# zhouxuguang/GNXRayTracer

Hardware: AMD Instinct MI355X
Metric: Mrays/sec + wall-clock to 1024spp, dragon Cornell 1920×1080 (higher is better)
Workload: dtype f32; 1 GPU; cfg3: Cornell + synthetic 100000-tri mesh (stand-in for absent dragon.3d), Glass+Metal, PathIntegrator maxDepth 8 rr 1 spatial, Halton(1024), 1920x1080; passes_in_flight=4, sub_passes=56, spp_rendered=1024, gather=n/a, world_size=1, backend=none, devices_visible=1

## Files before the change

gnxraytracer_amd/csrc/api_query.hip.h:

```cpp
#pragma once

extern "C" {


static const long long kQueryLaunchMax = 1ll << 30;

static DScene query_device_scene(gnxr_scene *r) {
    const CompiledScene &cs = r->cs;
    DScene sc = {};
    sc.nodes = reinterpret_cast<const float4 *>(r->nodes.p);
    sc.nodes4 = reinterpret_cast<const float4 *>(r->nodes4.p);
    sc.root4 = cs.root4;
    sc.tris = r->tris.p;
    sc.leaf_box = reinterpret_cast<const float4 *>(r->leaf_boxes.p);
    sc.leaf1_from_verts = (cs.leaf1_from_verts && !Knobs::leaf_box_table()) ? 1 : 0;
    sc.spheres = r->spheres.p;
    sc.n_spheres = cs.n_spheres;
    sc.materials = r->materials.p + 1;
    return sc;
}

static int query_trace4(gnxr_scene *r, const DScene &sc, const gnxr_ray *d_rays, int64_t n, gnxr_hit *hits, unsigned char *occluded, bool any, hipStream_t st) {
    const bool spheres = r->cs.n_spheres > 0;
    const TraceLaunch tl = trace_launch(r, true, spheres, std::min<long long>(n, kQueryLaunchMax));
    const size_t spill_ints = tl.spill_needed ? (size_t)(tl.entries - tl.lds_entries) * (size_t)tl.blocks * kBlock : 0;
    StreamScratch scratch;
    HIP_TRY(scratch.alloc(256 + spill_ints * sizeof(int), st));
    unsigned int *cursor = reinterpret_cast<unsigned int *>(scratch.p);
    int *spill = reinterpret_cast<int *>(scratch.p + 256);
    for (long long base = 0; base < n; base += kQueryLaunchMax) {
        const long long cnt = std::min<long long>(n - base, kQueryLaunchMax);
        const TraceLaunch t = trace_launch(r, true, spheres, cnt);
        QueryArrays qa;
        qa.rays = reinterpret_cast<const float4 *>(d_rays + base);
        qa.hits = any ? nullptr : hits + base;
        qa.occluded = any ? occluded + base : nullptr;
        TraceWork w = {};
        w.n_closest = (int)cnt;
        HIP_TRY(hipMemsetAsync(cursor, 0, sizeof(unsigned int), st));
#define GX_QUERY4(S, P, Q) hipLaunchKernelGGL((k_trace4<false, S, P, Q>), dim3(t.blocks), dim3(kBlock), t.lds, st, sc, qa, w, cursor, (Counters *)nullptr, t.lds_entries, spill, kTraceChunk, t.n_top)
#define GX_QUERY4_SP(Q) do { if (spheres) { if (t.spill_needed) GX_QUERY4(true, true, Q); else GX_QUERY4(true, false, Q); } \
                             else { if (t.spill_needed) GX_QUERY4(false, true, Q); else GX_QUERY4(false, false, Q); } } while (0)
        if (any) GX_QUERY4_SP(kT4QueryAny);
        else GX_QUERY4_SP(kT4QueryClosest);
#undef GX_QUERY4_SP
#undef GX_QUERY4
        HIP_TRY(hipGetLastError());
    }
    return GNXR_OK;
}

static int closest_hit_codes(gnxr_scene *r, const DScene &sc, const gnxr_ray *d_rays, long long n, gnxr_hit *codes, hipStream_t st) {
    if (r->wide_ok) return query_trace4(r, sc, d_rays, n, codes, nullptr, false, st);
    if (r->stack_size > 32) hipLaunchKernelGGL((k_trace_closest_code<64>), dim3(grid_for(n, 2)), dim3(kBlock), 0, st, sc, d_rays, n, codes);
    else hipLaunchKernelGGL((k_trace_closest_code<32>), dim3(grid_for(n, 5)), dim3(kBlock), 0, st, sc, d_rays, n, codes);
    HIP_TRY(hipGetLastError());
    return GNXR_OK;
}

static int trace_device(gnxr_scene *s, const gnxr_ray *d_rays, int64_t n, void *out, void *hip_stream, bool any) {
    if (!s || n < 0 || (n > 0 && (!d_rays || !out))) { set_error("bad argument"); return GNXR_ERR_INVALID; }
    if (n == 0) return GNXR_OK;
    if (((uintptr_t)d_rays & 15u) != 0) { set_error("d_rays is not 16-byte aligned (two dwordx4 loads per ray)"); return GNXR_ERR_INVALID; }
    if (!any && ((uintptr_t)out & 3u) != 0) { set_error("d_hits is not 4-byte aligned"); return GNXR_ERR_INVALID; }
    const QueryArg args[] = {{d_rays, (size_t)n * sizeof(gnxr_ray), "d_rays"}, {out, (size_t)n * (!any ? sizeof(gnxr_hit) : 1), !any ? "d_hits" : "d_occluded"}};
    DeviceCall call;
    int rc = call.bind(s, args);
    if (rc) return rc;
    gnxr_scene *r = call.r;
    hipStream_t st = (hipStream_t)hip_stream;
    const DScene sc = query_device_scene(r);
    if (!r->wide_ok) return binary_trace_api(r, sc, d_rays, n, out, any, st);
    if ((rc = query_trace4(r, sc, d_rays, n, any ? nullptr : (gnxr_hit *)out, any ? (unsigned char *)out : nullptr, any, st)) != GNXR_OK) return rc;
    if (!any) {
        hipLaunchKernelGGL(k_query_finish, dim3(grid_for(n)), dim3(kBlock), 0, st, sc, reinterpret_cast<const float4 *>(d_rays), (long long)n, (gnxr_hit *)out);
        HIP_TRY(hipGetLastError());
    }
    return GNXR_OK;
}
int gnxr_trace_closest_device(gnxr_scene *s, const gnxr_ray *d_rays, int64_t n, gnxr_hit *d_hits, void *hip_stream) {
    return trace_device(s, d_rays, n, d_hits, hip_stream, false);
}
int gnxr_trace_any_device(gnxr_scene *s, const gnxr_ray *d_rays, int64_t n, uint8_t *d_occluded, void *hip_stream) {
    return trace_device(s, d_rays, n, d_occluded, hip_stream, true);
}

int gnxr_li_device(gnxr_scene *s, const gnxr_render_params *p, const gnxr_ray *d_rays, const gnxr_li_sample *d_samples, int64_t n, float *d_L, void *hip_stream,
                   gnxr_stats *stats) {
    if (int rc = ensure_device()) return rc;
    if (!s || !p || n < 0 || (n > 0 && (!d_rays || !d_samples || !d_L))) { set_error("bad argument"); return GNXR_ERR_INVALID; }
    if (p->spp_begin != 0 || p->spp_end != 0) { set_error("Li for caller rays: spp_begin and spp_end must be 0 (the records name each ray's sample)"); return GNXR_ERR_INVALID; }
    if (int rc = check_unsharded(*p, "Li for caller rays", "the records name each ray's sample")) return rc;
    if (n == 0) { if (stats) memset(stats, 0, sizeof(*stats)); return GNXR_OK; }
    if ((((uintptr_t)d_rays | (uintptr_t)d_samples | (uintptr_t)d_L) & 15u) != 0) { set_error("d_rays, d_samples and d_L must be 16-byte aligned"); return GNXR_ERR_INVALID; }
    const QueryArg args[] = {{d_rays, (size_t)n * sizeof(gnxr_ray), "d_rays"}, {d_samples, (size_t)n * sizeof(gnxr_li_sample), "d_samples"}, {d_L, (size_t)n * 4 * sizeof(float), "d_L"}};
    DeviceCall call;
    if (int rc = call.bind(s, args)) return rc;
    gnxr_render_params pp = *p;
    pp.shard_count = 1; pp.shard_rows = 1;
    const RaySource src{d_rays, d_samples, d_L, (long long)n};
    return render_one(call.r, &pp, nullptr, hip_stream, stats, false, &src);
}

int gnxr_render_views_device(gnxr_scene *s, const gnxr_render_params *p, const gnxr_camera *cameras, const int32_t *camera_media, int32_t n_views, void *d_rgba_out,
                             void *hip_stream, gnxr_stats *stats) {
    if (!s || !p || n_views < 0 || (n_views > 0 && !cameras)) { set_error("bad argument"); return GNXR_ERR_INVALID; }
    if (int rc = check_unsharded(*p, "views", "a caller that shards splits the list of views")) return rc;
    if (!image_and_samples_ok(*p) || p->max_depth < 0 || p->max_depth > 250) return invalid_render_params();
    if (n_views == 0) { if (stats) memset(stats, 0, sizeof(*stats)); return GNXR_OK; }
    if (!d_rgba_out || ((uintptr_t)d_rgba_out & 15u) != 0) { set_error("d_rgba_out is null or not 16-byte aligned"); return GNXR_ERR_INVALID; }
    long long total = 0;
    if (int rc = check_view_pixels(p->width, p->height, n_views, "views", &total)) return rc;
    if (int rc = ensure_device()) return rc;
    if (int rc = check_view_media(s, camera_media, n_views, "views")) return rc;
    const QueryArg args[] = {{d_rgba_out, (size_t)total * sizeof(float4), "d_rgba_out"}};
    DeviceCall call;
    if (int rc = call.bind(s, args)) return rc;
    gnxr_render_params pp = *p;
    pp.shard_count = 1; pp.shard_rows = 1;
    const ViewSource vs{cameras, camera_media, (int)n_views};
    return render_one(call.r, &pp, d_rgba_out, hip_stream, stats, false, nullptr, &vs);
}


static const long long kBsdfQueryChunk = 1ll << 22;
// ... 94 lines not shown
```

gnxraytracer_amd/csrc/api_render.hip.h:

```cpp
#pragma once

struct TraceLaunch {
    int entries;
    int lds_entries;
    bool spill_needed;
    size_t lds;
    int n_top;
    int blocks;
};
static TraceLaunch trace_launch(const gnxr_scene *s, bool wide, bool spheres, long long total) {
    TraceLaunch t;
    t.entries = wide ? s->cs.stack4_need + 1 : s->cs.bvh_max_depth + 2;
    const int per_cu = g_trace_blocks_per_cu;
    const size_t fixed_b = wide ? (size_t)(kRayRecDwords + (spheres ? 1 : 0)) * kRqStride * sizeof(int) + (size_t)kTopCache * 128 + kOrderTableBytes : 0;
    t.lds_entries = std::min(std::min(t.entries, Knobs::trace_lds_levels()), std::max(2, (int)(((160 * 1024) / per_cu - 1024 - fixed_b) / (kBlock * sizeof(int)))));
    t.spill_needed = t.entries > t.lds_entries;
    t.lds = (size_t)t.lds_entries * kBlock * sizeof(int) + fixed_b;
    t.n_top = (int)std::min<size_t>(kTopCache, s->cs.root4 >= 0 ? s->cs.nodes4.size() : 0);
    t.blocks = (int)std::min<long long>((long long)g_num_cus * per_cu, (total + kBlock - 1) / kBlock);
    return t;
}

static int count_local_rows(const gnxr_render_params *p) {
    int rows = 0;
    for (int y = 0; y < p->height; ++y)
        if ((y / p->shard_rows) % p->shard_count == p->shard_index) ++rows;
    return rows;
}

struct RaySource {
    const gnxr_ray *rays;
    const gnxr_li_sample *samples;
    float *L;
    long long n;
};

struct ViewSource {
    const gnxr_camera *cameras;
    const int32_t *media;
    int n_views;
};

struct FilmSource {
    FilmFilter f;
    FilmTable tab;
    float4 *accum;
    bool keep;
};

static FilmImage film_image(int W, int H, int n_views) {
    FilmImage im;
    im.W = W; im.H = H;
    im.npix = (long long)n_views * W * H;
    im.tiles_x = (W + kFilmTile - 1) / kFilmTile;
    im.tiles_y = (H + kFilmTile - 1) / kFilmTile;
    im.n_tiles = (long long)n_views * im.tiles_y * im.tiles_x;
    return im;
}
static int film_grid(const FilmImage &im) { return grid_for(im.n_tiles * kBlock, 32); }

struct PixelListSource {
    gnxr_adaptive_params ap;
    int32_t *count_out;
    PixelRound round;
    int rounds;
    long long samples, at_budget;
};

constexpr int kAdaptiveGrowth = 8;
static int adaptive_round_samples(const gnxr_adaptive_params &ap, int spp, int n0) {
    return n0 == 0 ? ap.min_spp : std::min(std::max(ap.step_spp, n0 / kAdaptiveGrowth), spp - n0);
}

struct RenderPlan {
    gnxr_render_params p;
    bool direct, volpath, whitted;
    int wmode;
    int n_records, max_light_samples;
    bool textured_scene;
    int class_mask;
    bool area_only, area_env_only;
    bool escape_queue;
    int queue_kernel[4];
    unsigned kind_queue;
    bool caller_rays;
    int n_views;
    bool pixel_list;
    int local_rows, npix;
    long long unit, unit_begin, unit_end;
    int spill_entries;
    int k, in_flight;
    size_t half, cap, nrec;

    bool path_int() const { return !whitted && !volpath; }
    int nsamples() const { return p.spp_end - p.spp_begin; }
    int size_passes(size_t slots_held, bool have_mem, size_t free_b);
};

enum ShadeQueueKernel { SHADE_Q_NONE = 0, SHADE_Q_DIFFUSE, SHADE_Q_GLOSSY, SHADE_Q_CONDUCTOR, SHADE_Q_ROUGH_DIELECTRIC, SHADE_Q_ALL, SHADE_Q_TEX, SHADE_Q_ESCAPE };
// ... 211 lines not shown
    va.bind_records(rec_primary);
    va.mis_Y = mis_Y.p;
    va.vs = vol_vs.p; va.n1 = vol_n1.p; va.f = vol_f.p;
    va.Li = vol_Li.p; va.Tr = vol_Tr.p; va.Ld = vol_Ld.p; va.mres = vol_mres.p; va.state = vol_state.p;
    va.orig = vol_orig.p; va.Lout = vol_Lout.p;
    return va;
}
WhittedArrays RenderState::whitted_arrays(const RenderPlan &pl, int n_lights) {
    WhittedArrays wa;
    wa.ws = vol_vs.p; wa.fr_o = wh_o.p; wa.fr_d = wh_d.p; wa.fr_L = wh_L.p; wa.fr_w = wh_w.p; wa.fr_pdf = wh_pdf.p;
    wa.fr_rxo = wh_rxo.p; wa.fr_rxd = wh_rxd.p; wa.fr_ryo = wh_ryo.p; wa.fr_ryd = wh_ryd.p;
    wa.cap = (int)pl.cap; wa.n_lights = n_lights; wa.n_records = pl.n_records;
    wa.start_dim = pl.wmode == WM_DIRECT_ALL ? 5 + 2 * (pl.p.max_depth * n_lights * 2) : 5;
    return wa;
}
VolPackSet RenderState::pack_set(bool alt) {
    VolPackSet ps;
    if (!alt) {
        float4 *a[kVolPackF4] = {L.p, reinterpret_cast<float4 *>(vol_vs.p), vol_n1.p, vol_f.p, vol_Li.p, vol_Tr.p, vol_Ld.p, mis_Y.p, vol_mres.p};
        for (int i = 0; i < kVolPackF4; ++i) ps.f4[i] = a[i];
        record_ptrs(rec, ps.rec);
        ps.state = vol_state.p; ps.orig = vol_orig.p;
    } else {
        for (int i = 0; i < kVolPackF4; ++i) ps.f4[i] = vol_alt[i].p;
        record_ptrs(vol_alt_rec, ps.rec);
        ps.state = vol_alt_state.p; ps.orig = vol_alt_orig.p;
    }
    return ps;
}

struct RenderRun {
    gnxr_scene *s;
    RenderState &st;
    hipStream_t stream;
    const RenderPlan &pl;
    const RaySource *src;
    const ViewSource *views;
    const PixelListSource *pix;
    const FilmSource *film = nullptr;
    float4 *film_accum = nullptr;
    DScene sc;
    DRender r;
    PathArrays pa;
    VolArrays va;
    WhittedArrays wa;
    DMediaTables mt;
    Counters *dctr;
    KernelTimer timer;
    const bool timing = (g_profiling & 1) != 0, count_wide = (g_profiling & 4) != 0, counting = (g_profiling & 2) != 0 && !count_wide;
    bool spheres;
    const int mis_mode = Knobs::no_mis_defer() ? 0 : Knobs::mis_defer_step(), mis_drain_at = Knobs::mis_defer_drain_at();
    bool list_media = false;
    int n_lights, n_scene_media;
    unsigned long long rays_closest = 0, rays_any = 0, rays_mis = 0, media_segments = 0;
    unsigned long long new_paths = 0;
    unsigned int launches = 0, passes = 0, loop_iterations = 0;

    RenderRun(gnxr_scene *scene, hipStream_t stream_, const RenderPlan &plan, const RaySource *src_, const ViewSource *views_, const PixelListSource *pix_, const DScene &sc_,
              const DRender &r_)
        : s(scene), st(scene->st), stream(stream_), pl(plan), src(src_), views(views_), pix(pix_), sc(sc_), r(r_), pa(st.path_arrays()), va(st.vol_arrays()),
          wa(st.whitted_arrays(plan, (int)scene->cs.desc_lights.size())), mt(scene->media_tables()), dctr(scene->counters.p), spheres(scene->cs.n_spheres > 0),
          n_lights((int)scene->cs.desc_lights.size()), n_scene_media((int)scene->cs.media.size()) {}

    void launch_trace(TraceWork w, int n_sh, int n_mis, bool count_rays = true);
    void compact(int mode, const int *qin, int nin, const unsigned char *keys, int nout, int nscatter, unsigned int *totals, int *o0, int *o1, int *o2, int *o3 = nullptr, int split = 0,
                 const unsigned *n_dev = nullptr, unsigned kind_queue = 0x01010101u);
    int shade_stage(const int *q_in, int n, int *q_out, const unsigned *n_dev);
    void raygen(const PathArrays &at, long long u0, int kk, unsigned char *medium_keys);
    void resolve(const PathArrays &at, long long u0, int kk);
    void bind_set(const VolPackSet &ps);
};

void RenderRun::launch_trace(TraceWork w, int n_sh, int n_mis, bool count_rays) {
    long long total = (long long)w.n_closest + w.n_nee;
    if (total <= 0) return;
    w.order = nullptr;
    (void)hipMemsetAsync(&dctr->cursor, 0, sizeof(unsigned int), stream);
    const bool wide = s->wide_ok && !counting;
    const TraceLaunch tl = trace_launch(s, wide, spheres, total);
    if (timing) timer.begin(0, stream);
    const int chunk = Knobs::trace_chunk();
#define GX_TRACE(C, W, S) hipLaunchKernelGGL((k_trace<C, W, S>), dim3(tl.blocks), dim3(kBlock), tl.lds, stream, sc, pa, w, &dctr->cursor, dctr, tl.lds_entries, st.trace_spill.p, chunk)
#define GX_TRACE4(C, S, P) hipLaunchKernelGGL((k_trace4<C, S, P>), dim3(tl.blocks), dim3(kBlock), tl.lds, stream, sc, pa, w, &dctr->cursor, dctr, tl.lds_entries, st.trace_spill.p, chunk, tl.n_top)
#define GX_TRACE4_CS(C, S) do { if (tl.spill_needed) GX_TRACE4(C, S, true); else GX_TRACE4(C, S, false); } while (0)
    if (wide) {
        if (spheres) { if (count_wide) GX_TRACE4_CS(true, true); else GX_TRACE4_CS(false, true); }
        else { if (count_wide) GX_TRACE4_CS(true, false); else GX_TRACE4_CS(false, false); }
    } else {
        const bool cnt = counting || count_wide;
        if (spheres) { if (cnt) GX_TRACE(true, false, true); else GX_TRACE(false, false, true); }
        else { if (cnt) GX_TRACE(true, false, false); else GX_TRACE(false, false, false); }
    }
#undef GX_TRACE4_CS
#undef GX_TRACE4
#undef GX_TRACE
    if (timing) timer.end(stream);
    if (count_rays) {
        rays_closest += (unsigned long long)w.n_closest + (unsigned long long)n_mis;
        rays_any += (unsigned long long)n_sh;
        rays_mis += (unsigned long long)n_mis;
    }
    ++launches;
}

void RenderRun::compact(int mode, const int *qin, int nin, const unsigned char *keys, int nout, int nscatter, unsigned int *totals, int *o0, int *o1, int *o2, int *o3, int split,
                        const unsigned *n_dev, unsigned kind_queue) {
    const int tiles = (nin + kCompactTile - 1) / kCompactTile;
    const int g = std::max(1, std::min(tiles, g_num_cus * kCompactBlocksPerCu));
    if (st.compact_seq >= (1u << 30) - 1u) {
        (void)hipMemsetAsync(st.tile_desc.p, 0, st.tile_desc.n * sizeof(unsigned long long), stream);
        st.compact_seq = 0;
    }
    const unsigned seq = ++st.compact_seq;
    const CompactScratch cs{st.tile_desc.p, tiles, st.compact_ticket.p + (seq & 1u), st.compact_ticket.p + ((seq + 1u) & 1u), seq};
    const bool hitclass = mode == COMPACT_HITCLASS;
    const int *hit = hitclass ? (const int *)st.hit.p : nullptr;
    const unsigned char *cls = hitclass ? (const unsigned char *)s->tri_class.p : nullptr;
#define GX_COMPACT(M, N, NS) hipLaunchKernelGGL((k_compact<M, N, NS>), dim3(g), dim3(kCompactBlock), 0, stream, qin, nin, keys, cs, totals, o0, o1, o2, o3, hit, cls, kind_queue, split, n_dev, dctr)
    if (mode == COMPACT_FLAGS) {
        if (nout == 5) { if (nscatter == 3) GX_COMPACT(COMPACT_FLAGS, 5, 3); else GX_COMPACT(COMPACT_FLAGS, 5, 2); }
        else { if (nscatter == 3) GX_COMPACT(COMPACT_FLAGS, 4, 3); else GX_COMPACT(COMPACT_FLAGS, 4, 2); }
    } else if (hitclass) { if (nout == 4) GX_COMPACT(COMPACT_HITCLASS, 4, 4); else GX_COMPACT(COMPACT_HITCLASS, 3, 3); }
    else if (nout == 4) GX_COMPACT(COMPACT_CLASS, 4, 4);
    else GX_COMPACT(COMPACT_CLASS, 3, 3);
#undef GX_COMPACT
    launches += 1;
}
static int compact_stalled(const Counters &c) {
    if (!c.compact_stall) return GNXR_OK;
    set_error("queue compaction: a tile waited for its predecessors beyond the poll limit (k_compact); the render was abandoned");
    return GNXR_ERR_RUNTIME;
}

constexpr size_t kShadeLdsBudget = 52 * 1024;

int RenderRun::shade_stage(const int *q_in, int n, int *q_out, const unsigned *n_dev) {
    if (timing) timer.begin(2, stream);
    const int *qk = pl.queue_kernel;
    const int n_classes = qk[3] != SHADE_Q_NONE ? 4 : 3;
    compact(COMPACT_HITCLASS, q_in, n, st.pclass.p, n_classes, n_classes, &dctr->q_class[0], st.queue_c0.p, st.queue_c1.p, st.queue_c2.p, st.queue_c3.p, 0, n_dev, pl.kind_queue);
    int *qc[4] = {st.queue_c0.p, st.queue_c1.p, st.queue_c2.p, st.queue_c3.p};
    dim3 g(grid_for(n, Knobs::shade_blocks_per_cu())), b(kBlock);
    const int sdims = std::min<int>(Knobs::shade_lds_dims(), (int)s->cs.prime_sums.size() - 1);
    const int snperm = sdims > 0 ? s->cs.prime_sums[sdims] : 0;
    const bool shade_lds_tabs = Knobs::shade_lds_tables();
    const int lmats = (shade_lds_tabs && s->cs.materials.size() <= 12) ? (int)s->cs.materials.size() : 0;
    const int llights = (shade_lds_tabs && n_lights > 0 && n_lights <= 16) ? n_lights : 0;
    const size_t slds = (sdims > 0 ? ((((size_t)snperm * 2 + 15) & ~(size_t)15) + (size_t)sdims * 32) : 0) + (size_t)lmats * sizeof(DMaterial) + (size_t)llights * sizeof(DLight);
    const int shade_streams = Knobs::shade_streams();
    int n_class_kernels = 0;
    for (int q = 0; q < 4; ++q) n_class_kernels += qk[q] != SHADE_Q_NONE ? 1 : 0;
    const bool fork = (shade_streams < 0 ? n_class_kernels >= 3 : (shade_streams != 0 && n_class_kernels >= 2)) && s->aux_stream[0] && s->aux_stream[1];
    hipStream_t cst[4] = {stream, stream, stream, stream};
    if (fork) {
        HIP_TRY(hipEventRecord(s->ev_fork, stream));
        HIP_TRY(hipStreamWaitEvent(s->aux_stream[0], s->ev_fork, 0));
        HIP_TRY(hipStreamWaitEvent(s->aux_stream[1], s->ev_fork, 0));
        cst[1] = s->aux_stream[0]; cst[2] = s->aux_stream[1]; cst[3] = s->aux_stream[1];
    }
    const bool area_only = pl.area_only, area_env_only = pl.area_env_only;
#define GX_SHADE_KA(K, C, LDS, LL) hipLaunchKernelGGL(K, g, b, LDS, cst[C], sc, r, pa, (const int *)qc[C], (const unsigned int *)&dctr->q_class[C], sdims, snperm, lmats, LL)
#define GX_SHADE_K(K, C) GX_SHADE_KA(K, C, slds, llights)
#define GX_SHADE(LMV, LTV, C) do { if (spheres) GX_SHADE_K((k_shade<LMV, LTV, true>), C); else GX_SHADE_K((k_shade<LMV, LTV, false>), C); } while (0)
#define GX_SHADE_AREA_S(LMV, SPHV, C) do { \
        if (mis_step == 2) GX_SHADE_KA((k_shade<LMV, LT_AREA | SM_DEFER, SPHV>), C, slds_mis, llights_mis); \
        else if (mis_step == 1) GX_SHADE_K((k_shade<LMV, LT_AREA | SM_DIR_FIRST, SPHV>), C); \
        else GX_SHADE_K((k_shade<LMV, LT_AREA, SPHV>), C); } while (0)
// ... 554 lines not shown
```

gnxraytracer_amd/csrc/trace4_kernel.hip.h:

```cpp
#pragma once
#include "kernels.hip.h"
#include "query_kernel.hip.h"
#include "wide_collapse.h"

namespace gnxr {

GX_DEV unsigned order_entry(unsigned code, unsigned hm) {
    const unsigned byte = wide_order_byte(code);
    unsigned e = 0, n = 0;
    for (int i = 0; i < 4; ++i) {
        const unsigned slot = (byte >> (2 * i)) & 3u;
        if ((hm >> slot) & 1u) { e |= slot << (2u * n); ++n; }
    }
    return e;
}
constexpr int kOrderTableBytes = 256;
#ifndef GX_T4_CACHE
#define GX_T4_CACHE 64
#endif
constexpr int kTopCache = GX_T4_CACHE;
constexpr int kRayRecDwords = 11;
#ifndef GX_T4_RQ
#define GX_T4_RQ 64
#endif
constexpr int kRayQueue = GX_T4_RQ;
constexpr int kRqStride = (kBlock / 64) * kRayQueue;
#ifndef GX_T4_NEE_LAG
#define GX_T4_NEE_LAG 128
#endif
constexpr int kNeeLag = GX_T4_NEE_LAG;
#ifndef GX_T4_NEE_TAIL
#define GX_T4_NEE_TAIL 0
#endif
#ifndef GX_T4_NEE_BESIDE
#define GX_T4_NEE_BESIDE 0
#endif
static_assert(kNeeLag >= 64 && kNeeLag % 64 == 0, "the lagging items must lie behind the batch that is being set up");
GX_DEV int trace4_lds_dwords_per_thread(bool sph) { return kRayRecDwords + (sph ? 1 : 0); }

#ifndef GX_T4_WAVES
#define GX_T4_WAVES 5
#endif
#if GX_T4_WAVES > 0
#define GX_T4_BOUNDS __launch_bounds__(kBlock, GX_T4_WAVES)
#else
#define GX_T4_BOUNDS __launch_bounds__(kBlock)
#endif
template <bool COUNT, bool SPH, bool SPILL, int Q = kT4Render>
__global__ void GX_T4_BOUNDS k_trace4(DScene sc, typename Trace4Src<Q>::type pa, TraceWork w, unsigned int *cursor, Counters *ctr, int lds_entries, int *spill, int chunk, int n_top) {
    extern __shared__ int smem[];
    typedef __attribute__((address_space(3))) float lds_float;
    lds_int *const stk = (lds_int *)&smem[threadIdx.x];
    global_int *const spl = (global_int *)(spill + (size_t)blockIdx.x * kBlock + threadIdx.x);
    const int spillStride = (int)gridDim.x * kBlock;
    const int lane = __lane_id();
    lds_int *const rq = (lds_int *)&smem[lds_entries * kBlock + (threadIdx.x >> 6) * kRayQueue];
    trace_work_counts(w);
    const unsigned total = (unsigned)w.n_closest + (unsigned)w.n_nee;
    chunk = trace_chunk(total, chunk);
    const ChunkPlan plan = chunk_plan(total, (unsigned)chunk);
    const unsigned nWaves = gridDim.x * (kBlock / 64u), waveId = blockIdx.x * (kBlock / 64u) + (threadIdx.x >> 6);
    bool firstFetch = true;
#ifdef GX_TAIL_STAMP
    const unsigned tailFrom = total;
    bool tailSeen = false;
    if (Q == kT4Render && waveId == 0 && lane == 0) atomicMin(&g_tail[2], (unsigned long long)wall_clock64());
#endif
    const DTri *__restrict__ tris = sc.tris;
    const char *__restrict__ nb = reinterpret_cast<const char *>(sc.nodes4);
    typedef float f4v __attribute__((ext_vector_type(4)));
    typedef __attribute__((address_space(3))) f4v lds_f4;
    typedef __attribute__((address_space(3))) unsigned char lds_u8;
    lds_f4 *const topN = (lds_f4 *)&smem[lds_entries * kBlock + (kRayRecDwords + (SPH ? 1 : 0)) * kRqStride];
    lds_u8 *const lut = (lds_u8 *)(topN + 8 * kTopCache);
    {
        const f4v *gn = reinterpret_cast<const f4v *>(sc.nodes4);
        for (int i = threadIdx.x; i < n_top * 8; i += kBlock) topN[(i & 7) * kTopCache + (i >> 3)] = gn[i];
        if (threadIdx.x < kOrderTableBytes) lut[threadIdx.x] = (unsigned char)order_entry(threadIdx.x >> 4, threadIdx.x & 15u);
        __syncthreads();
    }

    auto push = [&](int &n, int v) {
        if (!SPILL || n < lds_entries) stk[n * kBlock] = v;
        else spl[(n - lds_entries) * spillStride] = v;
        ++n;
    };
    auto pop = [&](int &n) -> int {
        --n;
        return (!SPILL || n < lds_entries) ? stk[n * kBlock] : spl[(n - lds_entries) * spillStride];
    };

#ifndef GX_T4_REFILL_IN_A
#define GX_T4_REFILL_IN_A 0
#endif
    unsigned poolBase = 0, poolCount = 0;
    bool exhausted = false;
    unsigned rqHead = 0, rqCount = 0;
    unsigned nNeeApplied = 0;

    bool live = false;
    int pk = 0, path = -1;
    constexpr int kMisOwed = 256;
    V3 ro, inv;
    float Sx = 0, Sy = 0, tMax = 0;
    unsigned oNX = 0, oNY = 16, oNZ = 32;
    unsigned ordShift = 0;
    int cur = -1, toVisit = 0, leafOff = 0, leafN = 0, hitLeaf = -1;
    uint32_t cntNodes = 0, cntTris = 0, cntRetests = 0, cntNodesGlobal = 0;
#ifdef GX_TRACE_STATS
    unsigned long long st_[24] = {0};
#endif

    auto take_ray = [&](unsigned slot) {
        const lds_float *q = (const lds_float *)(rq + slot);
        ro = V3(q[0 * kRqStride], q[1 * kRqStride], q[2 * kRqStride]); tMax = q[3 * kRqStride];
        inv = V3(q[4 * kRqStride], q[5 * kRqStride], q[6 * kRqStride]); Sx = q[7 * kRqStride];
        Sy = q[8 * kRqStride];
        pk = (pk & kMisOwed) | __float_as_int(q[9 * kRqStride]);
        path = __float_as_int(q[10 * kRqStride]);
        hitLeaf = SPH ? rq[slot + 11 * kRqStride] : -1;
        const int neg0 = inv.x < 0, neg1 = inv.y < 0, neg2 = inv.z < 0;
        oNX = neg0 ? 48u : 0u; oNY = neg1 ? 64u : 16u; oNZ = neg2 ? 80u : 32u;
        ordShift = 4u * (unsigned)(neg0 | (neg1 << 1) | (neg2 << 2));
        cur = ((pk >> 4) & 1) ? -1 : sc.root4; toVisit = 0; leafN = 0;
        live = true;
    };
    auto retire_ray = [&]() {
        const int kind = pk & 3;
        if constexpr (Q == kT4QueryClosest) pa.hits[path].prim = hitLeaf;
        else if constexpr (Q == kT4QueryAny) pa.occluded[path] = hitLeaf != -1 ? 1 : 0;
        else if (kind == 0) {
            pa.hit[path] = hitLeaf;
            if (hitLeaf < 0) {
                int cls = sc.escape_class;
                if (SPH && hitLeaf != -1) { const int mat = sc.spheres[-2 - hitLeaf].material; if (mat >= 0) cls = sc.materials[mat].shade_class; }
                else if (sc.lt.n_infinite == 0) {
                    cls = 4;
                    pa.pflags[path] = 0;
                }
                pa.pclass[path] = (unsigned char)cls;
            }
        }
        else if (kind == 1) {
            if (w.vis) w.vis[4 * (size_t)path] = hitLeaf == -1 ? 3 : 2;
            else reinterpret_cast<float *>(&pa.sh_o[(size_t)path * kRS])[3] = hitLeaf == -1 ? 1.f : 0.f;
        } else {
            const int expect = __float_as_int(pa.mis_o[(size_t)path * kRS].w);
            bool ok = (expect >= 0) ? (hitLeaf == expect) : (hitLeaf == -1);
            if (w.vis) w.vis[4 * (size_t)path + 1] = ok ? 3 : 2;
            else reinterpret_cast<float *>(&pa.mis_o[(size_t)path * kRS])[3] = ok ? 1.f : 0.f;
        }
        live = false;
    };
    auto nee_round = [&](unsigned first, unsigned lo, unsigned hi) {
        if constexpr (Q == kT4Render) {
            __builtin_amdgcn_fence(__ATOMIC_SEQ_CST, "workgroup");
            const unsigned j = first + (unsigned)lane;
            bool did = false;
            if (j >= lo && j < hi) {
                const int p = w.q_nee[j - (unsigned)w.n_closest];
                unsigned *vw = reinterpret_cast<unsigned *>(w.vis) + p;
                const unsigned v = __hip_atomic_load(vw, __ATOMIC_RELAXED, __HIP_MEMORY_SCOPE_WAVEFRONT);
                if (nee_ready(v)) {
                    nee_apply(pa, p, v);
                    reinterpret_cast<unsigned char *>(vw)[3] = 1;
                    did = true;
                }
            }
            nNeeApplied += (unsigned)__popcll(__ballot(did));
        }
    };
#ifdef GX_TRACE_STATS
#define GX_TICK(i) do { const unsigned long long t_ = __builtin_amdgcn_s_memtime(); GX_STAT(i, t_ - tick_); tick_ = t_; } while (0)
// ... 78 lines not shown
                            }
                        }
                    }
                    unsigned neeV = 0;
#if GX_T4_NEE_BESIDE
                    float4 neeX = make_float4(0, 0, 0, 0), neeB = neeX, neeL = neeX;
#endif
                    if constexpr (Q == kT4Render) {
                        if (neeOn) {
                            __builtin_amdgcn_fence(__ATOMIC_SEQ_CST, "workgroup");
                            if (neeP >= 0) {
                                neeV = __hip_atomic_load(reinterpret_cast<unsigned *>(w.vis) + neeP, __ATOMIC_RELAXED, __HIP_MEMORY_SCOPE_WAVEFRONT);
#if GX_T4_NEE_BESIDE
                                neeX = pa.sh_X[(size_t)neeP * kRS]; neeB = pa.nbeta[(size_t)neeP * kRS]; neeL = pa.L[neeP];
#endif
                            }
                        }
                    }
                    {
                        if (valid) {
                            const V3 o(o4.x, o4.y, o4.z), d(d4.x, d4.y, d4.z);
                            const V3 iv(1.f / d.x, 1.f / d.y, 1.f / d.z);
                            const RayShear sh = ray_shear(d);
                            int done = 0;
                            for (int si = 0; SPH && si < sc.n_spheres; ++si) {
                                float tH;
                                if (sphere_test(sc.spheres[si], o, d, tMax_, &tH)) {
                                    sphHit = -2 - si;
                                    if (any_) { done = 1; break; }
                                    tMax_ = tH;
                                }
                            }
                            const int ex = (__builtin_isinf(iv.x) || __builtin_isinf(iv.y) || __builtin_isinf(iv.z)) ? 1 : 0;
                            r0 = make_float4(o.x, o.y, o.z, tMax_);
                            r1 = make_float4(iv.x, iv.y, iv.z, sh.Sx);
                            r2 = make_float4(sh.Sy, __int_as_float(kind_ | (sh.kz << 2) | (done << 4) | (ex << 5) | (any_ << 6)), __int_as_float(path_), 0.f);
                        }
                    }
                    const unsigned long long vm = __ballot(valid);
                    if (valid) {
                        const int slot = __popcll(vm & ((1ull << lane) - 1ull));
                        lds_float *q = (lds_float *)(rq + slot);
                        q[0 * kRqStride] = r0.x; q[1 * kRqStride] = r0.y; q[2 * kRqStride] = r0.z; q[3 * kRqStride] = r0.w;
                        q[4 * kRqStride] = r1.x; q[5 * kRqStride] = r1.y; q[6 * kRqStride] = r1.z; q[7 * kRqStride] = r1.w;
                        q[8 * kRqStride] = r2.x; q[9 * kRqStride] = r2.y; q[10 * kRqStride] = r2.z;
                        if (SPH) rq[slot + 11 * kRqStride] = sphHit;
                    }
                    __builtin_amdgcn_fence(__ATOMIC_SEQ_CST, "wavefront");
                    rqCount = (unsigned)__popcll(vm); rqHead = 0;
                    if constexpr (Q == kT4Render) {
                        if (neeOn) {
                            const bool did = neeP >= 0 && nee_ready(neeV);
                            if (did) {
#if GX_T4_NEE_BESIDE
                                if (nee_adds(neeV)) pa.L[neeP] = nee_sum(pa, neeP, neeV, neeX, neeB, neeL);
#else
                                nee_apply(pa, neeP, neeV);
#endif
                                reinterpret_cast<unsigned char *>(w.vis)[4 * (size_t)neeP + 3] = 1;
                            }
                            nNeeApplied += (unsigned)__popcll(__ballot(did));
                        }
                    }
                    bool advance = true;
                    if (Q == kT4Render) {
                        if (misPass) pk &= ~kMisOwed;
                        else if (wantMis) pk |= kMisOwed;
                        advance = misPass || __ballot(wantMis) == 0;
                    }
                    if (advance) { poolBase += take; poolCount -= take; }
                    GX_STAT(7, 1);
                    GX_STAT(8, misPass ? rqCount : take);
                }
            }
            if (rqCount > 0) {
                const unsigned rank = (unsigned)__popcll(needMask & ((1ull << lane) - 1ull));
                if (need && rank < rqCount) take_ray(rqHead + rank);
                const unsigned t = min(rqCount, (unsigned)__popcll(needMask));
                rqHead += t; rqCount -= t;
                __builtin_amdgcn_fence(__ATOMIC_SEQ_CST, "wavefront");
            }
        }
        GX_TICK(11);
        const unsigned long long liveMask = __ballot(live);
        if (liveMask == 0) {
            if (exhausted && rqCount == 0 && poolCount == 0) break;
            continue;
        }

        int nLive = __popcll(liveMask);
        GX_STAT(9, nLive);
        while (true) {
#if GX_T4_REFILL_IN_A
            {
                const bool fin = live && cur == -1 && leafN == 0;
                const unsigned long long finMask = __ballot(fin);
                if (finMask != 0 && rqCount > 0) {
                    if (fin) retire_ray();
                    const unsigned rank = (unsigned)__popcll(finMask & ((1ull << lane) - 1ull));
                    if (fin && rank < rqCount) take_ray(rqHead + rank);
                    const unsigned t = min(rqCount, (unsigned)__popcll(finMask));
                    rqHead += t; rqCount -= t;
                    __builtin_amdgcn_fence(__ATOMIC_SEQ_CST, "wavefront");
                    nLive = __popcll(__ballot(live));
                }
            }
#endif
            if (live && leafN == 0 && cur < -1) {
                const int lr = ~cur;
                leafOff = lr & 0xffffff; leafN = (lr >> 24) & 0x7f;
                cur = (toVisit == 0) ? -1 : pop(toVisit);
            }
            const bool searching = live && cur >= 0 && (kSpeculate || leafN == 0);
            const bool hungry = searching && leafN == 0;
            const int nSearching = __popcll(__ballot(hungry));
            if (nSearching * kTraceLeaveDiv <= nLive * kTraceLeaveMul && (nSearching == 0 || nSearching < nLive)) break;
#ifdef GX_TRACE_STATS
            { const int ns = __popcll(__ballot(searching)); GX_STAT(1, 1); GX_STAT(2, ns); const int nh_ = __popcll(__ballot(live && leafN > 0 && !searching)), nf_ = __popcll(__ballot(live && cur == -1 && leafN == 0)), nsp_ = __popcll(__ballot(searching && leafN > 0));
              GX_STAT(20, nLive); GX_STAT(21, nh_); GX_STAT(22, nf_); GX_STAT(23, nsp_);
              const int n16 = __popcll(__ballot(searching && cur < 16)), n64 = __popcll(__ballot(searching && cur < 64)), n256 = __popcll(__ballot(searching && cur < 256)), n1k = __popcll(__ballot(searching && cur < 1024));
              GX_STAT(16, n16); GX_STAT(17, n64); GX_STAT(18, n256); GX_STAT(19, n1k); }
#endif
            if (searching) {
                if (COUNT) cntNodes++;
                f4v nX, fX, nY, fY, nZ, fZ, cf;
                unsigned codes;
                if (cur < n_top) {
                    const lds_f4 *L = topN + cur;
                    nX = L[(oNX >> 4) * kTopCache]; fX = L[((48u - oNX) >> 4) * kTopCache];
                    nY = L[(oNY >> 4) * kTopCache]; fY = L[((80u - oNY) >> 4) * kTopCache];
                    nZ = L[(oNZ >> 4) * kTopCache]; fZ = L[((112u - oNZ) >> 4) * kTopCache];
                    cf = L[6 * kTopCache];
                    codes = __float_as_uint(L[7 * kTopCache].z);
                } else {
                    if (COUNT) cntNodesGlobal++;
                    const unsigned off = (unsigned)cur << 7;
#define GX_LD4(o) (*reinterpret_cast<const f4v *>(nb + (unsigned)(off + (o))))
                    nX = GX_LD4(oNX); fX = GX_LD4(48u - oNX); nY = GX_LD4(oNY); fY = GX_LD4(80u - oNY); nZ = GX_LD4(oNZ); fZ = GX_LD4(112u - oNZ);
                    cf = GX_LD4(96u);
                    codes = *reinterpret_cast<const unsigned *>(nb + (unsigned)(off + 120u));
#undef GX_LD4
                }
                const float k = 1 + 2 * GX_GAMMA(3);
                unsigned hitMask = 0;
                if (!(pk & 32)) {
#define GX_SLAB3(C, BIT)                                                                                       \
    {                                                                                                          \
        const float e = fmaxf(fmaxf((nX.C - ro.x) * inv.x, (nY.C - ro.y) * inv.y), (nZ.C - ro.z) * inv.z);      \
        const float x = fminf(fminf((fX.C - ro.x) * inv.x, (fY.C - ro.y) * inv.y), (fZ.C - ro.z) * inv.z) * k;  \
        hitMask |= (e <= x && e < tMax && x > 0.f) ? (BIT) : 0u;                                                \
    }
                    GX_SLAB3(x, 1u) GX_SLAB3(y, 2u) GX_SLAB3(z, 4u) GX_SLAB3(w, 8u)
#undef GX_SLAB3
                } else {
#define GX_SLAB(C, BIT)                                                                   \
    {                                                                                     \
        float tMin = (nX.C - ro.x) * inv.x, tMx = (fX.C - ro.x) * inv.x;                  \
        float tyMin = (nY.C - ro.y) * inv.y, tyMax = (fY.C - ro.y) * inv.y;               \
        tMx *= k; tyMax *= k;                                                             \
        bool ok = !(tMin > tyMax || tyMin > tMx);                                         \
        if (tyMin > tMin) tMin = tyMin;                                                   \
        if (tyMax < tMx) tMx = tyMax;                                                     \
        float tzMin = (nZ.C - ro.z) * inv.z, tzMax = (fZ.C - ro.z) * inv.z;               \
        tzMax *= k;                                                                       \
        ok = ok && !(tMin > tzMax || tzMin > tMx);                                        \
        if (tzMin > tMin) tMin = tzMin;                                                   \
        if (tzMax < tMx) tMx = tzMax;                                                     \
        ok = ok && (tMin < tMax) && (tMx > 0);                                            \
        hitMask |= ok ? (BIT) : 0u;                                                       \
    }
                    GX_SLAB(x, 1u) GX_SLAB(y, 2u) GX_SLAB(z, 4u) GX_SLAB(w, 8u)
#undef GX_SLAB
                }
                int next;
                if (hitMask == 0) next = (toVisit == 0) ? -1 : pop(toVisit);
                else {
                    const unsigned e = lut[(((codes >> ordShift) & 15u) << 4) | hitMask];
                    const int n = __popc(hitMask);
                    const int c0 = __float_as_int(cf.x), c1 = __float_as_int(cf.y), c2 = __float_as_int(cf.z), c3 = __float_as_int(cf.w);
                    auto child = [&](unsigned s) -> int { const int lo = (s & 1u) ? c1 : c0, hi = (s & 1u) ? c3 : c2; return (s & 2u) ? hi : lo; };
                    if (n >= 4) push(toVisit, child(e >> 6));
                    if (n >= 3) push(toVisit, child((e >> 4) & 3u));
                    if (n >= 2) push(toVisit, child((e >> 2) & 3u));
                    next = child(e & 3u);
                }
                cur = next;
            }
        }
        GX_TICK(12);
#ifdef GX_TRACE_STATS
        {
            unsigned long long lm = __ballot(live && leafN > 0);
            if (lm) {
                int mx = leafN;
                for (int o = 32; o > 0; o >>= 1) mx = max(mx, __shfl_xor(mx, o));
                int sm = live ? leafN : 0;
                for (int o = 32; o > 0; o >>= 1) sm += __shfl_xor(sm, o);
                const int nre = __popcll(__ballot(live && leafN > 0 && hitLeaf >= 0));
                GX_STAT(3, 1); GX_STAT(4, __popcll(lm)); GX_STAT(5, mx); GX_STAT(6, sm); GX_STAT(10, nre);
            }
        }
#endif
        if (live && leafN > 0) {
            bool visit = true;
            const bool first = (pk & 128) == 0;
            const bool retest = first && (SPH ? hitLeaf != -1 : hitLeaf >= 0);
            const bool fromVerts = retest && leafN == 1 && sc.leaf1_from_verts;
            int neg[3] = {inv.x < 0, inv.y < 0, inv.z < 0};
            if (retest && !fromVerts) {
                const float4 b0 = sc.leaf_box[2 * (size_t)leafOff], b1 = sc.leaf_box[2 * (size_t)leafOff + 1];
                if (COUNT) cntRetests++;
                visit = slab_test(b0, b1, ro, inv, neg, tMax);
            }
            bool more = false;
            if (visit) {
                RayShear shear;
                const int kz = (pk >> 2) & 3;
                shear.kz = kz; shear.kx = kz == 2 ? 0 : kz + 1; shear.ky = shear.kx == 2 ? 0 : shear.kx + 1;
                shear.Sx = Sx; shear.Sy = Sy; shear.Sz = kz == 0 ? inv.x : (kz == 1 ? inv.y : inv.z);
                V3 p0, p1, p2;
                load_tri(tris, leafOff, &p0, &p1, &p2);
#ifndef GX_COUNT_TRI_TESTS
                if (COUNT) cntTris++;
#endif
                bool inBox = true;
                if (fromVerts) {
                    const float4 b0 = make_float4(fminf(fminf(p0.x, p1.x), p2.x), fminf(fminf(p0.y, p1.y), p2.y), fminf(fminf(p0.z, p1.z), p2.z), fmaxf(fmaxf(p0.x, p1.x), p2.x));
                    const float4 b1 = make_float4(fmaxf(fmaxf(p0.y, p1.y), p2.y), fmaxf(fmaxf(p0.z, p1.z), p2.z), 0.f, 0.f);
                    inBox = slab_test(b0, b1, ro, inv, neg, tMax);
                }
                more = leafN > 1;
#ifdef GX_COUNT_TRI_TESTS
                if (COUNT && inBox) cntTris++;
#endif
                TriHit h;
                if (inBox && tri_test_sheared(p0, p1, p2, ro, shear, tMax, &h)) {
                    hitLeaf = leafOff;
                    if (pk & 64) { cur = -1; more = false; }
                    else tMax = h.t;
                }
            }
            if (more) { leafOff += 1; leafN -= 1; pk |= 128; }
            else { leafN = 0; pk &= ~128; }
        }
        GX_TICK(13);
        if (live && cur == -1 && leafN == 0) retire_ray();
    }
#ifdef GX_TRACE_STATS
    if (lane == 0) for (int i = 0; i < 24; ++i) if (st_[i]) atomicAdd(&g_trace_stats[i], st_[i]);
#endif
    if (Q == kT4Render && nNeeApplied != 0 && lane == 0) atomicAdd(&ctr->nee_applied_trace, (unsigned long long)nNeeApplied);
    if (COUNT) {
        atomicAdd(&ctr->nodes, (unsigned long long)cntNodes);
        atomicAdd(&ctr->tris, (unsigned long long)cntTris);
        atomicAdd(&ctr->retests, (unsigned long long)cntRetests);
        atomicAdd(&ctr->nodes_global, (unsigned long long)cntNodesGlobal);
    }
#ifdef GX_TAIL_STAMP
    if (Q == kT4Render && lane == 0) {
        atomicMax(&g_tail[1], (unsigned long long)wall_clock64());
        __threadfence();
        if (atomicAdd(&g_tail[3], 1ull) == (unsigned long long)nWaves - 1ull) {
            __threadfence();
            const unsigned long long tEnd = atomicExch(&g_tail[1], 0ull), tCross = atomicExch(&g_tail[0], ~0ull), tStart = atomicExch(&g_tail[2], ~0ull);
            atomicExch(&g_tail[3], 0ull);
            const unsigned long long behind = tEnd > tCross ? tEnd - tCross : 0ull, all = tEnd > tStart ? tEnd - tStart : 0ull;
            const int o = total >= (1u << 24) ? 8 : 4;
            g_tail[o] += behind; g_tail[o + 1] += all; g_tail[o + 2] += 1ull; g_tail[o + 3] += total;
// ... 8 lines not shown
```

gnxraytracer_amd/csrc/wide_collapse.h:

```cpp
#pragma once
#include <stdint.h>

#include "gnxr_device_types.h"

#if defined(__HIPCC__)
#define GX_WIDE_HD __host__ __device__ inline
#else
#define GX_WIDE_HD inline
#endif

namespace gnxr {

struct WideCost { float t[4]; };
static_assert(sizeof(WideCost) == 16, "WideCost is read as one dwordx4");

GX_WIDE_HD bool wide_is_leaf(const DNode &n) { return (n.meta & 0xffffu) != 0; }
GX_WIDE_HD int wide_axis(const DNode &n) { return (int)(n.meta >> 16) & 3; }

GX_WIDE_HD int wide_best_k(uint8_t choice) { return 2 + (choice & 3); }
GX_WIDE_HD int wide_split(uint8_t choice, int k) { return k == 2 ? 1 : (k == 3 ? 1 + ((choice >> 2) & 1) : 1 + ((choice >> 3) & 3)); }

GX_WIDE_HD float wide_area(const DNode &n) {
    const float dx = n.hi0 - n.lo[0], dy = n.hi1 - n.lo[1], dz = n.hi2 - n.lo[2];
    return 2.f * ((dx * dy + dy * dz) + dz * dx);
}

GX_WIDE_HD WideCost wide_cost_leaf() {
    WideCost c;
    c.t[0] = 0.f; c.t[1] = c.t[2] = c.t[3] = __builtin_inff();
    return c;
}
GX_WIDE_HD uint8_t wide_cost_interior(const DNode &X, const WideCost &a, const WideCost &b, WideCost *out) {
    const float t2 = a.t[0] + b.t[0];
    float t3 = a.t[0] + b.t[1];
    int i3 = 1;
    { const float c = a.t[1] + b.t[0]; if (c < t3) { t3 = c; i3 = 2; } }
    float t4 = a.t[0] + b.t[2];
    int i4 = 1;
    { const float c = a.t[1] + b.t[1]; if (c < t4) { t4 = c; i4 = 2; } }
    { const float c = a.t[2] + b.t[0]; if (c < t4) { t4 = c; i4 = 3; } }
    float m = t2;
    int k = 2;
    if (t3 < m) { m = t3; k = 3; }
    if (t4 < m) { m = t4; k = 4; }
    out->t[0] = wide_area(X) + m; out->t[1] = t2; out->t[2] = t3; out->t[3] = t4;
    return (uint8_t)((k - 2) | ((i3 - 1) << 2) | ((i4 - 1) << 3));
}

GX_WIDE_HD unsigned wide_order_byte(unsigned code) {
    unsigned o0, o1, o2, o3;
    if (!(code & 8u)) {
        const unsigned base0 = (code & 4u) ? 2u : 0u, base1 = 2u - base0, sw0 = (code >> 1) & 1u, sw1 = code & 1u;
        o0 = base0 + sw0; o1 = base0 + 1u - sw0; o2 = base1 + sw1; o3 = base1 + 1u - sw1;
    } else {
        const unsigned p0 = (code & 1u) ? 3u : 2u, p1 = 5u - p0;
        const unsigned r0 = (code & 2u) ? p0 : 1u, r1 = (code & 2u) ? p1 : p0, r2 = (code & 2u) ? 1u : p1;
        if (code & 4u) { o0 = r0; o1 = r1; o2 = r2; o3 = 0u; }
        else { o0 = 0u; o1 = r0; o2 = r1; o3 = r2; }
    }
    return o0 | (o1 << 2) | (o2 << 4) | (o3 << 6);
}

struct WideCut {
    int slot[4];
    int n;
    uint32_t codes;
    uint32_t order_lo, order_hi;
};
GX_WIDE_HD WideCut wide_cut(const DNode *bn, const uint8_t *choice, int bi) {
    WideCut c;
    c.slot[0] = c.slot[1] = c.slot[2] = c.slot[3] = -1;
    const DNode N = bn[bi];
    const int A = bi + 1, B = N.offset;
    const int k = wide_best_k(choice[bi]), i = wide_split(choice[bi], k), j = k - i;
    c.n = k;
    int ax0 = wide_axis(N), ax1 = 0, ax2 = 0, flip0 = 0, flip1 = 0;
    unsigned shape = 0u;
    if (i <= 2 && j <= 2) {
        if (i == 1) c.slot[0] = A; else { c.slot[0] = A + 1; c.slot[1] = bn[A].offset; ax1 = wide_axis(bn[A]); }
        if (j == 1) c.slot[2] = B; else { c.slot[2] = B + 1; c.slot[3] = bn[B].offset; ax2 = wide_axis(bn[B]); }
    } else {
        shape = 8u;
        const int M = i == 1 ? B : A;
        c.slot[0] = i == 1 ? A : B; flip0 = i == 1 ? 0 : 1;
        const DNode m = bn[M];
        const int i2 = wide_split(choice[M], 3);
        const int P = i2 == 1 ? m.offset : M + 1;
        c.slot[1] = i2 == 1 ? M + 1 : m.offset; flip1 = i2 == 1 ? 0 : 1;
        ax1 = wide_axis(m);
        c.slot[2] = P + 1; c.slot[3] = bn[P].offset; ax2 = wide_axis(bn[P]);
    }
    c.codes = 0u; c.order_lo = 0u; c.order_hi = 0u;
    for (int oct = 0; oct < 8; ++oct) {
        const int n0 = (oct >> ax0) & 1, n1 = (oct >> ax1) & 1, n2 = (oct >> ax2) & 1;
        unsigned code;
        if (!shape) {
            const int h = n0, a = h ? n2 : n1, b = h ? n1 : n2;
            code = (unsigned)((h << 2) | (a << 1) | b);
        } else code = 8u | (unsigned)(((n0 ^ flip0) << 2) | ((n1 ^ flip1) << 1) | n2);
        c.codes |= code << (4 * oct);
        const uint32_t byte = wide_order_byte(code);
        if (oct < 4) c.order_lo |= byte << (8 * oct); else c.order_hi |= byte << (8 * (oct - 4));
    }
    return c;
}

}
```

Measured before the change: 5403 Mrays/s.

## Push all wide-BVH children unconditionally and guard stack spills with wave-uniform checks

Reworks the 4-wide traversal stack handling. On a hit, three child slots are now written to the LDS stack without branching and the depth is advanced by n-1, using a new precomputed push-order table and two extra LDS stack levels of headroom. Spill-checked push/pop is selected per iteration by a wave-uniform ballot that tests whether any lane is near the LDS limit, and ballot/popcount control values are forced into scalar registers. The aim is to remove per-push divergence and spill checks in the common case, at the cost of more LDS per block (possible occupancy loss) and extra ballots per step.

```diff
diff --git a/gnxraytracer_amd/csrc/api_query.hip.h b/gnxraytracer_amd/csrc/api_query.hip.h
--- a/gnxraytracer_amd/csrc/api_query.hip.h
+++ b/gnxraytracer_amd/csrc/api_query.hip.h
@@ -39,8 +39,8 @@
         w.n_closest = (int)cnt;
         HIP_TRY(hipMemsetAsync(cursor, 0, sizeof(unsigned int), st));
 #define GX_QUERY4(S, P, Q) hipLaunchKernelGGL((k_trace4<false, S, P, Q>), dim3(t.blocks), dim3(kBlock), t.lds, st, sc, qa, w, cursor, (Counters *)nullptr, t.lds_entries, spill, kTraceChunk, t.n_top)
-#define GX_QUERY4_SP(Q) do { if (spheres) { if (t.spill_needed) GX_QUERY4(true, true, Q); else GX_QUERY4(true, false, Q); } \
-                             else { if (t.spill_needed) GX_QUERY4(false, true, Q); else GX_QUERY4(false, false, Q); } } while (0)
+#define GX_QUERY4_SP(Q) do { if (spheres) { if (t.checked) GX_QUERY4(true, true, Q); else GX_QUERY4(true, false, Q); } \
+                             else { if (t.checked) GX_QUERY4(false, true, Q); else GX_QUERY4(false, false, Q); } } while (0)
         if (any) GX_QUERY4_SP(kT4QueryAny);
         else GX_QUERY4_SP(kT4QueryClosest);
 #undef GX_QUERY4_SP
diff --git a/gnxraytracer_amd/csrc/api_render.hip.h b/gnxraytracer_amd/csrc/api_render.hip.h
--- a/gnxraytracer_amd/csrc/api_render.hip.h
+++ b/gnxraytracer_amd/csrc/api_render.hip.h
@@ -4,6 +4,7 @@
     int entries;
     int lds_entries;
     bool spill_needed;
+    bool checked;
     size_t lds;
     int n_top;
     int blocks;
@@ -13,8 +14,10 @@
     t.entries = wide ? s->cs.stack4_need + 1 : s->cs.bvh_max_depth + 2;
     const int per_cu = g_trace_blocks_per_cu;
     const size_t fixed_b = wide ? (size_t)(kRayRecDwords + (spheres ? 1 : 0)) * kRqStride * sizeof(int) + (size_t)kTopCache * 128 + kOrderTableBytes : 0;
-    t.lds_entries = std::min(std::min(t.entries, Knobs::trace_lds_levels()), std::max(2, (int)(((160 * 1024) / per_cu - 1024 - fixed_b) / (kBlock * sizeof(int)))));
+    const int want = t.entries + (wide ? kStackHeadroom : 0);
+    t.lds_entries = std::min(std::min(want, Knobs::trace_lds_levels()), std::max(2, (int)(((160 * 1024) / per_cu - 1024 - fixed_b) / (kBlock * sizeof(int)))));
     t.spill_needed = t.entries > t.lds_entries;
+    t.checked = t.lds_entries < want;
     t.lds = (size_t)t.lds_entries * kBlock * sizeof(int) + fixed_b;
     t.n_top = (int)std::min<size_t>(kTopCache, s->cs.root4 >= 0 ? s->cs.nodes4.size() : 0);
     t.blocks = (int)std::min<long long>((long long)g_num_cus * per_cu, (total + kBlock - 1) / kBlock);
@@ -392,7 +395,7 @@
     const int chunk = Knobs::trace_chunk();
 #define GX_TRACE(C, W, S) hipLaunchKernelGGL((k_trace<C, W, S>), dim3(tl.blocks), dim3(kBlock), tl.lds, stream, sc, pa, w, &dctr->cursor, dctr, tl.lds_entries, st.trace_spill.p, chunk)
 #define GX_TRACE4(C, S, P) hipLaunchKernelGGL((k_trace4<C, S, P>), dim3(tl.blocks), dim3(kBlock), tl.lds, stream, sc, pa, w, &dctr->cursor, dctr, tl.lds_entries, st.trace_spill.p, chunk, tl.n_top)
-#define GX_TRACE4_CS(C, S) do { if (tl.spill_needed) GX_TRACE4(C, S, true); else GX_TRACE4(C, S, false); } while (0)
+#define GX_TRACE4_CS(C, S) do { if (tl.checked) GX_TRACE4(C, S, true); else GX_TRACE4(C, S, false); } while (0)
     if (wide) {
         if (spheres) { if (count_wide) GX_TRACE4_CS(true, true); else GX_TRACE4_CS(false, true); }
         else { if (count_wide) GX_TRACE4_CS(true, false); else GX_TRACE4_CS(false, false); }
diff --git a/gnxraytracer_amd/csrc/trace4_kernel.hip.h b/gnxraytracer_amd/csrc/trace4_kernel.hip.h
--- a/gnxraytracer_amd/csrc/trace4_kernel.hip.h
+++ b/gnxraytracer_amd/csrc/trace4_kernel.hip.h
@@ -1,20 +1,30 @@
 #pragma once
+#include <type_traits>
+
 #include "kernels.hip.h"
 #include "query_kernel.hip.h"
 #include "wide_collapse.h"
 
 namespace gnxr {
 
-GX_DEV unsigned order_entry(unsigned code, unsigned hm) {
-    const unsigned byte = wide_order_byte(code);
-    unsigned e = 0, n = 0;
-    for (int i = 0; i < 4; ++i) {
-        const unsigned slot = (byte >> (2 * i)) & 3u;
-        if ((hm >> slot) & 1u) { e |= slot << (2u * n); ++n; }
-    }
-    return e;
+#ifndef GX_T4_STACK_GUARD
+#define GX_T4_STACK_GUARD 1
+#endif
+#ifndef GX_T4_PUSH_ALL
+#define GX_T4_PUSH_ALL 1
+#endif
+#ifndef GX_T4_SCALAR_CTRL
+#define GX_T4_SCALAR_CTRL 1
+#endif
+GX_DEV unsigned order_entry(unsigned code, unsigned hm) { return GX_T4_PUSH_ALL ? wide_push_entry(code, hm) : wide_order_entry(code, hm); }
+constexpr int kOrderTableBytes = 256;
+GX_DEV unsigned long long t4_ballot(bool b) { return __builtin_amdgcn_ballot_w64(b); }
+GX_DEV unsigned t4_count(unsigned long long mask) {
+    unsigned n = (unsigned)__builtin_popcountll(mask);
+    asm("" : "+s"(n));
+    return n;
 }
-constexpr int kOrderTableBytes = 256;
+constexpr int kStackHeadroom = GX_T4_PUSH_ALL ? 2 : 0;
 #ifndef GX_T4_CACHE
 #define GX_T4_CACHE 64
 #endif
@@ -80,15 +90,16 @@
         __syncthreads();
     }
 
-    auto push = [&](int &n, int v) {
-        if (!SPILL || n < lds_entries) stk[n * kBlock] = v;
+    auto push = [&](auto ck, int &n, int v) {
+        if (!decltype(ck)::value || n < lds_entries) stk[n * kBlock] = v;
         else spl[(n - lds_entries) * spillStride] = v;
         ++n;
     };
-    auto pop = [&](int &n) -> int {
+    auto pop = [&](auto ck, int &n) -> int {
         --n;
-        return (!SPILL || n < lds_entries) ? stk[n * kBlock] : spl[(n - lds_entries) * spillStride];
+        return (!decltype(ck)::value || n < lds_entries) ? stk[n * kBlock] : spl[(n - lds_entries) * spillStride];
     };
+    typedef std::integral_constant<bool, SPILL> stack_checked;
 
 #ifndef GX_T4_REFILL_IN_A
 #define GX_T4_REFILL_IN_A 0
@@ -333,13 +344,17 @@
             }
         }
         GX_TICK(11);
-        const unsigned long long liveMask = __ballot(live);
+        const unsigned long long liveMask = GX_T4_SCALAR_CTRL ? t4_ballot(live) : __ballot(live);
         if (liveMask == 0) {
             if (exhausted && rqCount == 0 && poolCount == 0) break;
             continue;
         }
 
+#if GX_T4_SCALAR_CTRL
+        unsigned nLive = t4_count(liveMask);
+#else
         int nLive = __popcll(liveMask);
+#endif
         GX_STAT(9, nLive);
         while (true) {
 #if GX_T4_REFILL_IN_A
@@ -353,20 +368,37 @@
                     const unsigned t = min(rqCount, (unsigned)__popcll(finMask));
                     rqHead += t; rqCount -= t;
                     __builtin_amdgcn_fence(__ATOMIC_SEQ_CST, "wavefront");
+#if GX_T4_SCALAR_CTRL
+                    nLive = t4_count(t4_ballot(live));
+#else
                     nLive = __popcll(__ballot(live));
-                }
-            }
+#endif
+                }
+            }
+#endif
+#if GX_T4_STACK_GUARD
+            unsigned nDeep = SPILL ? t4_count(t4_ballot(toVisit + 3 > lds_entries)) : 0u;
+#else
+            unsigned nDeep = SPILL ? 1u : 0u;
 #endif
             if (live && leafN == 0 && cur < -1) {
                 const int lr = ~cur;
                 leafOff = lr & 0xffffff; leafN = (lr >> 24) & 0x7f;
-                cur = (toVisit == 0) ? -1 : pop(toVisit);
+                if (toVisit == 0) cur = -1;
+                else if (nDeep == 0u) cur = pop(std::false_type(), toVisit);
+                else cur = pop(std::true_type(), toVisit);
             }
             const bool searching = live && cur >= 0 && (kSpeculate || leafN == 0);
             const bool hungry = searching && leafN == 0;
+#if GX_T4_SCALAR_CTRL
+            const unsigned nSearching = t4_count(t4_ballot(cur >= 0) & t4_ballot(leafN == 0));
+            if (nSearching * (unsigned)kTraceLeaveDiv <= nLive * (unsigned)kTraceLeaveMul && (nSearching == 0u || nSearching < nLive)) break;
+#else
             const int nSearching = __popcll(__ballot(hungry));
             if (nSearching * kTraceLeaveDiv <= nLive * kTraceLeaveMul && (nSearching == 0 || nSearching < nLive)) break;
+#endif
 #ifdef GX_TRACE_STATS
+            GX_STAT(14, nDeep == 0u ? 0 : 1);
             { const int ns = __popcll(__ballot(searching)); GX_STAT(1, 1); GX_STAT(2, ns); const int nh_ = __popcll(__ballot(live && leafN > 0 && !searching)), nf_ = __popcll(__ballot(live && cur == -1 && leafN == 0)), nsp_ = __popcll(__ballot(searching && leafN > 0));
               GX_STAT(20, nLive); GX_STAT(21, nh_); GX_STAT(22, nf_); GX_STAT(23, nsp_);
               const int n16 = __popcll(__ballot(searching && cur < 16)), n64 = __popcll(__ballot(searching && cur < 64)), n256 = __popcll(__ballot(searching && cur < 256)), n1k = __popcll(__ballot(searching && cur < 1024));
@@ -423,18 +455,36 @@
                     GX_SLAB(x, 1u) GX_SLAB(y, 2u) GX_SLAB(z, 4u) GX_SLAB(w, 8u)
 #undef GX_SLAB
                 }
-                int next;
-                if (hitMask == 0) next = (toVisit == 0) ? -1 : pop(toVisit);
-                else {
+                auto descend = [&](auto ck) -> int {
+                    if (hitMask == 0) return (toVisit == 0) ? -1 : pop(ck, toVisit);
                     const unsigned e = lut[(((codes >> ordShift) & 15u) << 4) | hitMask];
                     const int n = __popc(hitMask);
                     const int c0 = __float_as_int(cf.x), c1 = __float_as_int(cf.y), c2 = __float_as_int(cf.z), c3 = __float_as_int(cf.w);
                     auto child = [&](unsigned s) -> int { const int lo = (s & 1u) ? c1 : c0, hi = (s & 1u) ? c3 : c2; return (s & 2u) ? hi : lo; };
-                    if (n >= 4) push(toVisit, child(e >> 6));
-                    if (n >= 3) push(toVisit, child((e >> 4) & 3u));
-                    if (n >= 2) push(toVisit, child((e >> 2) & 3u));
-                    next = child(e & 3u);
-                }
+#if GX_T4_PUSH_ALL
+                    if constexpr (!decltype(ck)::value) {
+                        lds_int *const top = stk + toVisit * kBlock;
+                        top[0] = child(e & 3u); top[kBlock] = child((e >> 2) & 3u); top[2 * kBlock] = child((e >> 4) & 3u);
+                        toVisit += n - 1;
+                    } else {
+                        if (n >= 2) push(ck, toVisit, child(e & 3u));
+                        if (n >= 3) push(ck, toVisit, child((e >> 2) & 3u));
+                        if (n >= 4) push(ck, toVisit, child((e >> 4) & 3u));
+                    }
+                    return child(e >> 6);
+#else
+                    if (n >= 4) push(ck, toVisit, child(e >> 6));
+                    if (n >= 3) push(ck, toVisit, child((e >> 4) & 3u));
+                    if (n >= 2) push(ck, toVisit, child((e >> 2) & 3u));
+                    return child(e & 3u);
+#endif
+                };
+                int next;
+                if constexpr (SPILL && GX_T4_STACK_GUARD != 0) {
+                    asm("" : "+s"(nDeep));
+                    next = nDeep == 0u ? descend(std::false_type()) : descend(std::true_type());
+                }
+                else next = descend(stack_checked());
                 cur = next;
             }
         }
diff --git a/gnxraytracer_amd/csrc/wide_collapse.h b/gnxraytracer_amd/csrc/wide_collapse.h
--- a/gnxraytracer_amd/csrc/wide_collapse.h
+++ b/gnxraytracer_amd/csrc/wide_collapse.h
@@ -61,6 +61,28 @@
     return o0 | (o1 << 2) | (o2 << 4) | (o3 << 6);
 }
 
+GX_WIDE_HD unsigned wide_order_entry(unsigned code, unsigned hm) {
+    const unsigned byte = wide_order_byte(code);
+    unsigned e = 0, n = 0;
+    for (int i = 0; i < 4; ++i) {
+        const unsigned slot = (byte >> (2 * i)) & 3u;
+        if ((hm >> slot) & 1u) { e |= slot << (2u * n); ++n; }
+    }
+    return e;
+}
+GX_WIDE_HD unsigned wide_push_entry(unsigned code, unsigned hm) {
+    const unsigned e = wide_order_entry(code, hm);
+    unsigned n = 0;
+    for (int i = 0; i < 4; ++i) n += (hm >> i) & 1u;
+    if (n == 0) return 0u;
+    unsigned f[3], last = e & 3u;
+    for (unsigned i = 0; i < 3; ++i) {
+        if (i + 1 < n) last = (e >> (2u * (n - 1u - i))) & 3u;
+        f[i] = last;
+    }
+    return f[0] | (f[1] << 2) | (f[2] << 4) | ((e & 3u) << 6);
+}
+
 struct WideCut {
     int slot[4];
     int n;
```

Result: no change. 5433 Mrays/s, median of 6 (+0.6%).
